# MiniXC/LightningFastSpeech2

Hardware: AMD Instinct MI355X
Metric: mel-frames/sec (whole node), 256-phoneme batch-32 (higher is better)
Workload: dtype bf16

## Files before the change

include/fs2.h:

```cpp
#ifndef FS2_H_
#define FS2_H_

#include <stddef.h>
#include <stdint.h>

#ifdef __cplusplus
extern "C" {
#endif

#define FS2_ABI_VERSION 4
#define FS2_MAX_LAYERS 32
#define FS2_MAX_VARIANCES 4
#define FS2_MAX_PRIORS 8
#define FS2_NAME_LEN 32

enum fs2_status {
    FS2_OK = 0,
    FS2_ERR_HIP = 1,
    FS2_ERR_SHAPE = 2,
    FS2_ERR_ARG = 3,
    FS2_ERR_WEIGHT = 4,
    FS2_ERR_STATE = 5,
    FS2_ERR_NOMEM = 6
};
// ... 77 lines not shown
int fs2_set_graphs(fs2_engine* e, int32_t on);
int64_t fs2_graph_replays(const fs2_engine* e);
int fs2_set_deferred_layernorm(fs2_engine* e, int32_t on);
int fs2_set_folded_layernorm(fs2_engine* e, int32_t on);
int fs2_set_tuning(fs2_engine* e, int32_t knob);
int fs2_force_buckets(fs2_engine* e, int32_t variance_index, const int32_t* idx_device);
int fs2_force_variance_targets(fs2_engine* e, int32_t variance_index, const float* target_device);
int fs2_debug_copy(fs2_engine* e, const char* what, void* dst_device, void* hip_stream);

enum fs2_kernel_class {
    FS2_K_CONV_GEMM = 0,
    FS2_K_GEMM = 1,
    FS2_K_ATTENTION = 2,
    FS2_K_ROWOPS = 3,
    FS2_K_DEC_FFN_CONV1 = 4,
    FS2_K_DEC_ATTENTION = 5,
    FS2_K_ENC_MHA = 6,
    FS2_K_PREDICTOR = 7,
    FS2_K_COUNT = 8
};
int fs2_profile_enable(fs2_engine* e, int32_t kernel_class, int32_t enable);
int fs2_profile_reserve(fs2_engine* e, int32_t kernel_class, int32_t pairs);
int fs2_profile_read(fs2_engine* e, int32_t kernel_class, double* total_ms, int64_t* launches,
                     double* flops, double* bytes);

int fs2_op_set_gemm_variant(int32_t variant);
int fs2_op_set_vocoder_lds_limit(int32_t kib);
int fs2_op_set_vocoder_fused_resblock(int32_t on);
int32_t fs2_op_vocoder_resblock_form(int32_t dtype, int32_t channels, int32_t taps, const int32_t* dilations, int32_t npairs);
int32_t fs2_op_vocoder_conv_tile(int32_t dtype, int32_t n, int32_t cin, int32_t taps, int32_t dil, int32_t shift, int32_t post,
                                 int32_t* cin_pad);
int fs2_op_gemm(int32_t dtype, int32_t out_dtype, const void* x, const void* w, const float* bias, void* c,
                int32_t M, int32_t N, int32_t Cin, int32_t taps, int32_t S, int32_t relu, void* hip_stream);
int fs2_op_gemm_relu_dropout(int32_t dtype, const void* x, const void* w, const float* bias, void* c, int32_t M, int32_t N, int32_t Cin,
                             int32_t taps, int32_t S, float p, uint64_t seed, uint64_t key, void* hip_stream);
int fs2_op_gemm_add(int32_t dtype, const void* x, const void* w, const float* bias, const void* addend, void* c, int32_t M, int32_t N,
                    int32_t Cin, int32_t taps, int32_t S, void* hip_stream);
int fs2_op_gemm_rowscale(const void* x, const void* w, const float* bias, const float* rowstats, const float* wg,
                         void* c, int32_t M, int32_t N, int32_t Cin, void* hip_stream);
int fs2_op_gemm_rowscale_dt(int32_t dtype, int32_t out_dtype, const void* x, const void* w, const float* bias, const float* rowstats,
                            const float* wg, void* c, int32_t M, int32_t N, int32_t Cin, void* hip_stream);
int fs2_op_gemm_stats(int32_t dtype, const void* x, const void* w, const float* bias, const void* res, void* c, float* stats, int32_t M,
                      int32_t N, int32_t Cin, int32_t relu, void* hip_stream);
int fs2_op_rowstats_finish(const float* parts, int32_t nparts, int32_t ncols, float eps, float* out, int32_t M, void* hip_stream);
int fs2_op_gemm_head(const void* x, const void* w, const float* bias, const float* head_gw, float* stats_out, float* head_out, int32_t M,
                     int32_t N, int32_t Cin, int32_t relu, void* hip_stream);
int fs2_op_head_finish(const float* parts, const float* dots, int32_t nparts, int32_t ncols, float eps, float sum_gw, float cst,
                       const uint8_t* mask, float* pred, int32_t M, void* hip_stream);
int fs2_op_gemm_splitk_choice(int32_t dtype, int32_t M, int32_t N, int32_t Cin, int32_t taps, int32_t S);
int32_t fs2_op_gemm_route(int32_t dtype, int32_t out_dtype, int32_t M, int32_t N, int32_t Cin, int32_t taps, int32_t S, int32_t ksplit,
                          uint32_t present, int32_t bias_aligned);
int fs2_op_gemm_splitk(int32_t dtype, int32_t out_dtype, const void* x, const void* w, void* c, float* part, int32_t M, int32_t N,
                       int32_t Cin, int32_t taps, int32_t S, int32_t ksplit, int32_t accumulate, void* hip_stream);
int fs2_op_gemm_gated(int32_t dtype, const void* x, const void* w, const float* bias, const void* gate, float scale, void* c,
                      int32_t M, int32_t N, int32_t Cin, int32_t taps, int32_t S, void* hip_stream);
int fs2_op_attention(int32_t dtype, const void* qkv, const uint8_t* key_pad_mask, void* out, void* vt_scratch,
                     uint64_t* bits_scratch, int32_t B, int32_t S, int32_t H, int32_t heads, void* hip_stream);
int fs2_op_attention_x3(const float* qkv, const uint8_t* key_pad_mask, float* out, void* split_scratch, uint64_t* bits_scratch,
                        int32_t B, int32_t S, int32_t H, int32_t heads, void* hip_stream);
int fs2_op_gemm_split_out(const void* x, const void* w, const float* bias, void* c_hi, void* c_lo, int32_t M, int32_t N, int32_t Cin,
                          int32_t split, void* hip_stream);
int fs2_op_gemm_ln(int32_t dtype, const void* x, const void* w, const float* bias, const void* res,
                   const float* ln_g, const float* ln_b, const float* dot_w, float dot_b, const uint8_t* mask,
                   float* pred, void* y, void* tmp, int32_t M, int32_t N, int32_t Cin, int32_t taps, int32_t S,
                   int32_t relu, void* hip_stream);
int fs2_op_gemm_ln_tape(int32_t dtype, const void* x, const void* w, const float* bias, const void* res, const float* ln_g,
// ... 251 lines not shown
```

lightningfastspeech2_amd/csrc/capi_ops.hip:

```cpp
#include <math.h>

#include "fs2_common.h"
#include "fs2_kernels.h"

using namespace fs2;

namespace fs2 {

template <typename S, typename D>
__global__ __launch_bounds__(256) void convert_kernel(const S* __restrict__ s, D* __restrict__ d, size_t n) {
    for (size_t i = (size_t)blockIdx.x * 256 + threadIdx.x; i < n; i += (size_t)gridDim.x * 256)
        d[i] = Num<D>::from_f32(Num<S>::to_f32(s[i]));
}

int launch_convert(const ConvertArgs& a, int sdt, int ddt, hipStream_t st) {
    if (a.n == 0) return FS2_OK;
    size_t blocks = (a.n + 255) / 256;
    if (blocks > 4096) blocks = 4096;
    const dim3 g((unsigned)blocks), b(256);
    if (sdt == FS2_F32 && ddt == FS2_F32) hipLaunchKernelGGL((convert_kernel<float, float>), g, b, 0, st, (const float*)a.src, (float*)a.dst, a.n);
    else if (sdt == FS2_F32 && ddt == FS2_BF16) hipLaunchKernelGGL((convert_kernel<float, bf16>), g, b, 0, st, (const float*)a.src, (bf16*)a.dst, a.n);
    else if (sdt == FS2_BF16 && ddt == FS2_F32) hipLaunchKernelGGL((convert_kernel<bf16, float>), g, b, 0, st, (const bf16*)a.src, (float*)a.dst, a.n);
    else if (sdt == FS2_BF16 && ddt == FS2_BF16) hipLaunchKernelGGL((convert_kernel<bf16, bf16>), g, b, 0, st, (const bf16*)a.src, (bf16*)a.dst, a.n);
    else if (sdt == FS2_F32 && ddt == FS2_F16) hipLaunchKernelGGL((convert_kernel<float, f16>), g, b, 0, st, (const float*)a.src, (f16*)a.dst, a.n);
    else if (sdt == FS2_F16 && ddt == FS2_F32) hipLaunchKernelGGL((convert_kernel<f16, float>), g, b, 0, st, (const f16*)a.src, (float*)a.dst, a.n);
    else if (sdt == FS2_F16 && ddt == FS2_F16) hipLaunchKernelGGL((convert_kernel<f16, f16>), g, b, 0, st, (const f16*)a.src, (f16*)a.dst, a.n);
    else return FS2_ERR_ARG;
    return hipGetLastError() == hipSuccess ? FS2_OK : FS2_ERR_HIP;
}

}

namespace fs2 {
int apply_knob(Tuning& t, int variant) {
    int ok = 1;
    if (variant == 1500 || variant == 1501) t.attn_x3 = variant - 1500;
    else if (variant >= 1400 && variant <= 1402) t.gemm_wres = variant - 1400;
    else if (variant == 1340 || variant == 1341) t.enc_attn_out = variant - 1340;
    else if (variant == 1320 || variant == 1321) t.pred_fuse_embed = variant - 1320;
    else if (variant >= 1200 && variant <= 1204) t.attn_pipe = variant - 1200;
    else if (variant == 1100 || variant == 1101) t.colsum_fused = variant - 1100;
    else if (variant == 1000 || variant == 1001) t.bgemm_tn256 = variant - 1000;
    else if (variant >= 905 && variant <= 908) { if (variant >= 907) t.attn_bwd_nb_dq = 3 + ((variant - 905) & 1); else t.attn_bwd_nb = 3 + ((variant - 905) & 1); }
    else if (variant == 909) t.attn_bwd_nb = 1;
    else if (variant >= 900 && variant <= 903) { if (variant >= 902) t.attn_bwd_nb_dq = ((variant - 900) & 1) + 1; else t.attn_bwd_nb = ((variant - 900) & 1) + 1; }
    else if (variant == 904) t.attn_bwd_nb_dq = 0;
    else if (variant == 800 || variant == 801) t.bgemm_full = variant - 800;
    else if (variant == 700 || variant == 701) t.bgemm_xcd = variant - 700;
    else if (variant == 500 || variant == 501) t.split_f32 = variant - 500;
    else if (variant == 230 || variant == 231) t.head_sums = variant - 230;
    else if (variant == 220 || variant == 221) t.gemm_persist = variant - 220;
    else if (variant >= 200 && variant <= 202) t.slab_xcd_remap = variant - 200;
    else if (variant >= 0 && variant <= 7 && variant != 2) t.gemm_variant = variant;
    else ok = 0;
    if (!ok) return FS2_ERR_ARG;
    ++t.gen;
    return FS2_OK;
}
Tuning& op_tuning() {
    static thread_local Tuning t;
    return t;
}
}

static GemmArgs gemm_args(const void* x, const void* w, const float* bias, void* c, int M, int N, int Cin, int taps, int S, int relu) {
    GemmArgs a;
    a.X = x; a.W = w; a.bias = bias; a.C = c;
    a.M = M; a.N = N; a.K = taps * Cin; a.ldx = Cin; a.ldc = N;
    a.Cin = Cin; a.taps = taps; a.pad = (taps - 1) / 2; a.S = S; a.relu = relu;
// ... 58 lines not shown
size_t fs2_op_masked_loss_ws_bytes(void) { return fs2::masked_loss_ws_bytes(); }

int fs2_op_masked_loss(const float* pred, const void* truth, int32_t truth_kind, const uint8_t* pad_mask, int64_t rows,
                       int32_t inner, int32_t kind, void* ws, float* out2, void* stream) {
    if (!pred || !truth || !pad_mask || !ws || !out2) return FS2_ERR_ARG;
    if ((kind != 0 && kind != 1) || (truth_kind != 0 && truth_kind != 1)) return FS2_ERR_ARG;
    fs2::LossArgs a;
    a.pred = pred; a.truth = truth; a.mask = pad_mask; a.ws = ws; a.out = out2;
    a.rows = rows; a.inner = inner; a.kind = kind; a.truth_kind = truth_kind;
    return fs2::launch_masked_loss(a, (hipStream_t)stream);
}

int fs2_op_set_vocoder_fused_resblock(int32_t on) {
    const bool defined = on == 0 || on == 1 || on == 2 || on == 4 || on == 7 || on == 9 || (on >= 50 && on <= 100);
    if (!defined) return FS2_ERR_ARG;
    fs2::op_tuning().voc_fused_resblock = on;
    return FS2_OK;
}

int fs2_op_set_vocoder_lds_limit(int32_t kib) {
    if (kib < 0 || kib > 150) return FS2_ERR_ARG;
    fs2::op_tuning().voc_lds_limit = kib;
    return FS2_OK;
}



int fs2_op_set_gemm_variant(int32_t variant) { return fs2::apply_knob(fs2::op_tuning(), variant); }

int fs2_op_gemm(int32_t dtype, int32_t out_dtype, const void* x, const void* w, const float* bias, void* c,
                int32_t M, int32_t N, int32_t Cin, int32_t taps, int32_t S, int32_t relu, void* stream) {
    GemmArgs a = gemm_args(x, w, bias, c, M, N, Cin, taps, S, relu);
    return launch_gemm(a, dtype, out_dtype, (hipStream_t)stream);
}

int fs2_op_gemm_relu_dropout(int32_t dtype, const void* x, const void* w, const float* bias, void* c, int32_t M, int32_t N, int32_t Cin,
                             int32_t taps, int32_t S, float p, uint64_t seed, uint64_t key, void* stream) {
    if (!(p > 0.f && p < 1.f)) return FS2_ERR_ARG;
    GemmArgs a = gemm_args(x, w, bias, c, M, N, Cin, taps, S, 1);
    a.drop_p = p; a.drop_seed = seed; a.drop_key = key;
    return launch_gemm(a, dtype, dtype, (hipStream_t)stream);
}

int fs2_op_gemm_add(int32_t dtype, const void* x, const void* w, const float* bias, const void* addend, void* c, int32_t M, int32_t N,
                    int32_t Cin, int32_t taps, int32_t S, void* stream) {
    if (!addend) return FS2_ERR_ARG;
    GemmArgs a = gemm_args(x, w, bias, c, M, N, Cin, taps, S, 0);
    a.epi_res = addend;
    if (N < 192 || M % S || !(taps & 1)) return FS2_ERR_SHAPE;
    return launch_gemm(a, dtype, dtype, (hipStream_t)stream);
}

int fs2_op_gemm_stats(int32_t dtype, const void* x, const void* w, const float* bias, const void* res, void* c, float* stats, int32_t M,
                      int32_t N, int32_t Cin, int32_t relu, void* stream) {
    if (!x || !w || !c || !stats) return FS2_ERR_ARG;
    GemmArgs a = gemm_args(x, w, bias, c, M, N, Cin, 1, M, relu);
    a.epi_res = res; a.stats_out = stats; a.ln_eps = 1e-5f;
    if (N < 192) return FS2_ERR_SHAPE;
    return launch_gemm(a, dtype, dtype, (hipStream_t)stream);
}

int fs2_op_gemm_rowscale(const void* x, const void* w, const float* bias, const float* rowstats, const float* wg,
                         void* c, int32_t M, int32_t N, int32_t Cin, void* stream) {
    return fs2_op_gemm_rowscale_dt(FS2_BF16, FS2_BF16, x, w, bias, rowstats, wg, c, M, N, Cin, stream);
}
int fs2_op_gemm_rowscale_dt(int32_t dtype, int32_t out_dtype, const void* x, const void* w, const float* bias, const float* rowstats,
// ... 474 lines not shown
```

lightningfastspeech2_amd/csrc/fs2_kernels.h:

```cpp
#pragma once
#include <hip/hip_runtime.h>
#include <stdint.h>

#include <type_traits>

#include "../../include/fs2.h"

namespace fs2 {

inline bool is_16bit(int dt) { return dt == FS2_BF16 || dt == FS2_F16; }
inline bool is_storage_dtype(int dt) { return dt == FS2_F32 || is_16bit(dt); }
inline bool is_f32_or_bf16(int dt) { return dt == FS2_F32 || dt == FS2_BF16; }
inline size_t elem_bytes(int dt) { return is_16bit(dt) ? 2 : 4; }

struct Tuning {
    int gemm_variant = 0;
    int gemm_wres = 1;
    int head_sums = 1;
    int gemm_persist = 1;
    int slab_xcd_remap = 1;
    int split_f32 = 0;
    int attn_pipe = 3;
    int attn_x3 = 1;
    int enc_attn_out = 1;
    int pred_fuse_embed = 1;
    int attn_bwd_nb = 1, attn_bwd_nb_dq = 0;
    int colsum_fused = 0;
    int bgemm_full = 1, bgemm_xcd = 1, bgemm_tn256 = 1;
    int voc_lds_limit = 0;
    int voc_fused_resblock = 1;
    unsigned long long gen = 0;
};
Tuning& op_tuning();
int apply_knob(Tuning& t, int variant);
inline const Tuning& tuning_of(const Tuning* t) { return t ? *t : op_tuning(); }

struct GemmArgs {
    const void* X;
    const void* W;
    const float* bias;
    void* C;
    void* C_lo = nullptr;
    int M, N, K;
    int ldx, ldc;
    int Cin, taps, pad;
    int S;
    int relu;
    const void* res = nullptr;
    const float* ln_g = nullptr;
    const float* ln_b = nullptr;
// ... 8 lines not shown
    const Tuning* tune = nullptr;
    const void* epi_res = nullptr;
    const float* epi_res_stats = nullptr;
    const float* epi_res_g = nullptr;
    const float* epi_res_b = nullptr;
    int epi_res_parts = 0;
    float* stats_out = nullptr;
    int w_presplit = 0;
    int split = 0;
    const uint8_t* zero_rows = nullptr;
    const void* gate = nullptr;
    float gate_scale = 1.f;
    float drop_p = 0.f;
    uint64_t drop_seed = 0, drop_key = 0;
    const float* rs_stats = nullptr;
    const float* rs_wg = nullptr;
    const float* head_gw = nullptr;
    float* head_out = nullptr;
    int ksplit = 0;
};
enum GemmFeature : unsigned {
    GF_BIAS = 1u << 0, GF_RES = 1u << 1, GF_LN = 1u << 2, GF_DOT = 1u << 3, GF_ZOUT = 1u << 4, GF_LNTMP = 1u << 5, GF_STATS = 1u << 6,
    GF_EPIRES = 1u << 7, GF_GATE = 1u << 8, GF_DROP = 1u << 9, GF_RS = 1u << 10 , GF_HEAD = 1u << 11 ,
    GF_ZR = 1u << 12, GF_CLO = 1u << 13, GF_SPLIT = 1u << 14, GF_WPRE = 1u << 15, GF_RELU = 1u << 16,
};
enum GemmFamily { GEMM_NONE = 0, GEMM_FLAT128 = 1, GEMM_SLAB = 2, GEMM_PERSIST = 3, GEMM_WRES = 4 };
struct GemmRoute {
    int status = FS2_OK;
    int family = GEMM_NONE;
    int mi = 0;
    int in_dtype = 0, out_dtype = 0;
    bool ln = false, split = false, defer = false, xpre = false;
    bool zr = false;
    bool two_launch = false;
    bool presplit = false;
};
inline bool layernorm_rows_ok(int H) { return H % 4 == 0 && H <= 1024; }
GemmRoute route_gemm(const GemmArgs& a, int in_dtype, int out_dtype);
int launch_route(const GemmRoute& r, const GemmArgs& a, hipStream_t stream);
inline int launch_gemm(const GemmArgs& a, int in_dtype, int out_dtype, hipStream_t stream) {
    return launch_route(route_gemm(a, in_dtype, out_dtype), a, stream);
}
int launch_presplit_pack(const float* w, void* out, size_t n_values, hipStream_t stream);
bool gemm_presplit_eligible(int N, int K);
int launch_split_k_reduce(const float* part, void* out, size_t n, int ksplit, int accumulate, int out_dtype, hipStream_t stream);
int gemm_splitk_choice(int M, int N, int Cin, int taps, int S, int in_dtype);
bool gemm_wres_supported(const GemmArgs& a, int in_dtype, int out_dtype, bool force);
int launch_gemm_wres(const GemmArgs& a, int dtype, hipStream_t stream);
bool gemm_persist_supported(const GemmArgs& a, int in_dtype, int out_dtype, int mi);
bool gemm_head_supported(const GemmArgs& a, int in_dtype, int out_dtype);
bool gemm_persist_pays(const GemmArgs& a, int mi);
int launch_gemm_persist(const GemmArgs& a, int dtype, int mi, hipStream_t stream);

struct AttnArgs {
    const void* qkv;
    void* vt;
    const uint64_t* kbits;
    void* out;
    int B, S, H, heads, Spad, nw64;
    float scale_log2e;
    const void* qkv_lo = nullptr;
    float* lse2 = nullptr;
    float drop_p = 0.f;
    uint64_t drop_seed = 0, drop_key = 0;
    const Tuning* tune = nullptr;
};
struct AttnOutArgs {
    const void* qkv;
    const uint64_t* kbits;
    const void* wpk;
    const float* bias;
    const void* res;
    const float* ln_g;
    const float* ln_b;
    void* out;
    int B, S, H, heads, nw64;
    float scale_log2e, eps;
};
bool attn_out_ln_supported(int dtype, int H, int heads, int S);
int launch_attn_out_ln(const AttnOutArgs& a, int dtype, hipStream_t stream);
struct AttnBwdArgs {
// ... 495 lines not shown
```

lightningfastspeech2_amd/csrc/gemm_mfma.hip:

```cpp
#include <string.h>

#include "fs2_common.h"
#include "fs2_kernels.h"

namespace fs2 {

static constexpr int BM = 128, BN = 128, ROWB = 128;
static constexpr int TILE_BYTES = BM * ROWB;

__device__ inline int swz(int row, int slot) { return row * ROWB + ((slot ^ (row & 7)) << 4); }

template <typename T, typename OutT, bool ZR = false>
__global__ __launch_bounds__(256) void gemm_conv_kernel(GemmArgs p) {
    extern __shared__ __attribute__((aligned(16))) unsigned char smem[];
    unsigned char* sX = smem;
    unsigned char* sW = smem + 2 * TILE_BYTES;
    constexpr int E16 = Num<T>::kPer16B;
    constexpr int KE = ROWB / (int)sizeof(T);

    const int tid = threadIdx.x, lane = tid & 63, wave = tid >> 6;
    const int tiles_n = (p.N + BN - 1) / BN;
    const int bm = blockIdx.x / tiles_n, bn = blockIdx.x % tiles_n;
    const int m0 = bm * BM, n0 = bn * BN;

// ... 1059 lines not shown
            mi = best;
        }
    }
    if (ln && family != GEMM_SLAB) return r;
    if (!rules_hold(q, subject, family)) return GemmRoute{FS2_ERR_SHAPE};
    r.family = family; r.mi = mi;
    if (family == GEMM_FLAT128) {
        r.zr = q.feats & GF_ZR;
        if (!(dtype_pair(in_dtype, out_dtype) & flat_dtypes(r.zr))) return GemmRoute{FS2_ERR_SHAPE};
    } else if (family == GEMM_SLAB) {
        r.ln = ln; r.defer = defer;
        if (!(dtype_pair(in_dtype, out_dtype) & slab_dtypes(ln, defer))) return GemmRoute{FS2_ERR_SHAPE};
        r.split = in_dtype == FS2_F32 && out_dtype == FS2_F32 && (q.have & ND_SPLIT_ON);
        r.xpre = r.split && a.taps > 1;
        r.presplit = r.split && !a.w_presplit;
    }
    return r;
}

static GemmRoute route_request(const GemmArgs& a, int in_dtype, int out_dtype) {
    const auto no = [](int status) { return GemmRoute{status}; };
    const auto on = [](int family, int mi) { GemmRoute r; r.family = family; r.mi = mi; return r; };
    if (!is_storage_dtype(in_dtype) || !is_storage_dtype(out_dtype)) return no(FS2_ERR_ARG);
    if ((in_dtype == FS2_F16 || out_dtype == FS2_F16) && (a.drop_p > 0.f || a.gate || a.z_out || a.ksplit > 1 || a.head_out || a.C_lo)) return no(FS2_ERR_ARG);
    const Tuning& tn = tuning_of(a.tune);
    if (a.head_out) {
        if (a.ln_g || !gemm_head_supported(a, in_dtype, out_dtype)) return no(FS2_ERR_SHAPE);
        return on(GEMM_PERSIST, 6);
    }
    if (!a.ln_g) {
        if (a.drop_p > 0.f) {
            if (!rules_hold(classify(a, in_dtype, out_dtype), GF_DROP, GEMM_NONE)) return no(FS2_ERR_SHAPE);
        } else if (tn.gemm_wres && tn.gemm_variant == 0 && a.ksplit <= 1 && gemm_wres_supported(a, in_dtype, out_dtype, tn.gemm_wres == 2)) {
            return on(GEMM_WRES, 0);
        }
        return route_one(a, in_dtype, out_dtype);
    }
    if (a.z_out && a.N > S_BN) return no(FS2_ERR_SHAPE);
    if (a.drop_p > 0.f && (a.N > S_BN || !a.z_out)) return no(FS2_ERR_SHAPE);
    if (a.N <= S_BN && in_dtype == out_dtype) {
        const GemmRoute r = route_one(a, in_dtype, out_dtype);
        if (r.status != FS2_OK || r.family != GEMM_NONE) return r;
    }
    if (a.z_out) return no(FS2_ERR_SHAPE);
    if (!a.ln_tmp || in_dtype != out_dtype) return no(FS2_ERR_ARG);
    GemmArgs g = a;
    g.ln_g = nullptr;
    g.C = a.ln_tmp;
    GemmRoute r = route_one(g, in_dtype, out_dtype);
    if (r.status != FS2_OK || r.family == GEMM_NONE) return r;
    if (!layernorm_rows_ok(a.N)) return no(FS2_ERR_SHAPE);
    r.two_launch = true;
    return r;
}
GemmRoute route_gemm(const GemmArgs& a, int in_dtype, int out_dtype) {
    GemmRoute r = route_request(a, in_dtype, out_dtype);
    r.in_dtype = in_dtype; r.out_dtype = out_dtype;
    return r;
}

template <int MI, bool LN, bool DEFER>
static int launch_slab_e(const GemmRoute& r, const GemmArgs& a, hipStream_t stream) {
    return with_dtypes<slab_dtypes(LN, DEFER)>(r.in_dtype, r.out_dtype, [&](auto t, auto o) {
        using T = typename decltype(t)::type;
        using OutT = typename decltype(o)::type;
        if constexpr (sizeof(T) == 4) {
            if (r.xpre) return launch_slab_t<T, OutT, MI, LN, true, DEFER, true>(a, stream);
            if (r.split) return launch_slab_t<T, OutT, MI, LN, true, DEFER>(a, stream);
        }
        return launch_slab_t<T, OutT, MI, LN, false, DEFER>(a, stream);
    });
}
template <int MI>
static int launch_slab_mi(const GemmRoute& r, const GemmArgs& a, hipStream_t stream) {
    if constexpr (MI <= 6) {
        if (r.ln) return launch_slab_e<MI, true, false>(r, a, stream);
        if (r.defer) return launch_slab_e<MI, false, true>(r, a, stream);
    }
    return launch_slab_e<MI, false, false>(r, a, stream);
}
template <bool ZR>
static int launch_flat(const GemmRoute& r, const GemmArgs& a, hipStream_t stream) {
    return with_dtypes<flat_dtypes(ZR)>(r.in_dtype, r.out_dtype, [&](auto t, auto o) {
        return launch_t<typename decltype(t)::type, typename decltype(o)::type, ZR>(a, stream);
    });
}

int launch_route(const GemmRoute& r, const GemmArgs& a_in, hipStream_t stream) {
    if (r.status != FS2_OK || r.family == GEMM_NONE) return r.status;
    GemmArgs a = a_in;
    if (r.two_launch) { a.ln_g = nullptr; a.C = a_in.ln_tmp; }
    void* tmp = nullptr;
    if (r.presplit) {
        const int st = presplit_on_the_fly(a, stream, &tmp);
        if (st != FS2_OK) { if (tmp) (void)hipFreeAsync(tmp, stream); return st; }
    }
    int st;
    if (r.family == GEMM_FLAT128) st = r.zr ? launch_flat<true>(r, a, stream) : launch_flat<false>(r, a, stream);
    else if (r.family == GEMM_PERSIST) st = launch_gemm_persist(a, r.in_dtype, r.mi, stream);
    else if (r.family == GEMM_WRES) st = launch_gemm_wres(a, r.in_dtype, stream);
    else if (r.mi == 1) st = launch_slab_mi<1>(r, a, stream);
    else if (r.mi == 2) st = launch_slab_mi<2>(r, a, stream);
    else if (r.mi == 4) st = launch_slab_mi<4>(r, a, stream);
    else if (r.mi == 6) st = launch_slab_mi<6>(r, a, stream);
    else st = launch_slab_mi<8>(r, a, stream);
    if (tmp) (void)hipFreeAsync(tmp, stream);
    if (st != FS2_OK || !r.two_launch) return st;
    LayerNormArgs l;
    l.x = a_in.ln_tmp; l.res = a_in.res; l.gamma = a_in.ln_g; l.beta = a_in.ln_b; l.y = a_in.C;
    l.dot_w = a_in.dot_w; l.dot_b = a_in.dot_b; l.mask = a_in.mask; l.pred = a_in.pred;
    l.M = a_in.M; l.H = a_in.N; l.eps = a_in.ln_eps;
    return launch_layernorm(l, r.out_dtype, stream);
}

bool gemm_presplit_eligible(int N, int K) { return N >= 192 && K % 32 == 0; }

__global__ __launch_bounds__(256) void presplit_pack_kernel(const float* w, unsigned char* out, size_t npairs) {
    const size_t i = (size_t)blockIdx.x * 256 + threadIdx.x;
    if (i >= npairs) return;
    const size_t chunk = i >> 2;
    const int sl = (int)(i & 3);
    const uint4 c0 = *(const uint4*)(w + chunk * 32 + 4 * sl), c1 = *(const uint4*)(w + chunk * 32 + 16 + 4 * sl);
    uint4 h, l;
    split_bf16x3(c0, c1, h, l);
    *(uint4*)(out + chunk * 128 + sl * 16) = h;
    *(uint4*)(out + chunk * 128 + (4 + sl) * 16) = l;
}
int launch_presplit_pack(const float* w, void* out, size_t n_values, hipStream_t stream) {
    if (n_values % 32) return FS2_ERR_SHAPE;
    if (!n_values) return FS2_OK;
    const size_t np = n_values / 8;
    hipLaunchKernelGGL(presplit_pack_kernel, dim3((unsigned)((np + 255) / 256)), dim3(256), 0, stream, w, (unsigned char*)out, np);
    return hipGetLastError() == hipSuccess ? FS2_OK : FS2_ERR_HIP;
// ... 58 lines not shown
```

lightningfastspeech2_amd/csrc/gemm_wres.hip:

```cpp
#include <hip/hip_runtime.h>

#include <type_traits>

#include "fs2_common.h"
#include "fs2_kernels.h"

namespace fs2 {
namespace {

constexpr int WR_K = 256, WR_ROWB = WR_K * 2, WR_MI = 3, WR_RT = 2 * WR_MI * 16;
constexpr int WR_TILEB = WR_RT * WR_ROWB;
__attribute__((unused)) constexpr int WR_NDMA = WR_TILEB / 1024 / 8;

__device__ __attribute__((unused)) inline int wr_wcol(int ni, int fgq) { return (ni >> 1) * 32 + fgq * 8 + (ni & 1) * 4; }

#ifdef FS2_WRES_PROBE
__device__ unsigned long long g_wres_stamps[2][64];
#define WRES_STAMP(i)                                                                                                      \
    do {                                                                                                                   \
        if (blockIdx.x == 0 && (threadIdx.x == 0 || threadIdx.x == 448) && (i) < 64)                                        \
            g_wres_stamps[threadIdx.x ? 1 : 0][i] = __builtin_amdgcn_s_memtime();                                           \
    } while (0)
#else
#define WRES_STAMP(i) do { } while (0)
#endif

template <typename T>
__global__ __launch_bounds__(512) void gemm_wres_kernel(GemmArgs p, int ncol, int nrg, int tiles) {
#if defined(__HIP_DEVICE_COMPILE__)
    __shared__ __attribute__((aligned(16))) unsigned char xs0[WR_TILEB];
    __shared__ __attribute__((aligned(16))) unsigned char xs1[WR_TILEB];
    const int tid = threadIdx.x, lane = tid & 63;
    const int wave = __builtin_amdgcn_readfirstlane(tid >> 6);
    const int wm = wave >> 2, wn = wave & 3, fr = lane & 15, fg = lane >> 4;
    const int xcd = blockIdx.x & 7, q = blockIdx.x >> 3;
    const int ct = q % ncol, rg = (q / ncol) * 8 + xcd;
    if (rg >= nrg) return;
    const int tbeg = (int)((long)rg * tiles / nrg), tend = (int)((long)(rg + 1) * tiles / nrg);
    if (tbeg >= tend) return;
    const int n0 = ct * 256;
    WRES_STAMP(0);

    uint4 fw[8][4];
    {
        const __amdgpu_buffer_rsrc_t wrs =
            __builtin_amdgcn_make_buffer_rsrc((void*)p.W, 0, (unsigned)((size_t)p.N * WR_K * 2), 0x00020000);
        auto wswz = [](int row) { return ((row >> 1) & 1) | (((row >> 3) & 3) << 1); };
        auto stage = [&](int cc0) {
#pragma unroll
            for (int c = 0; c < 2; ++c)
#pragma unroll
                for (int i = 0; i < 4; ++i) {
                    const int P = (i * 8 + wave) * 64 + lane, row = P >> 3, ps = P & 7;
                    const unsigned voff = (unsigned)((n0 + row) * (WR_K * 2) + (cc0 + c) * 128 + ((ps ^ wswz(row)) << 4));
                    __builtin_amdgcn_raw_ptr_buffer_load_lds(wrs, (__attribute__((address_space(3))) void*)((c ? xs1 : xs0) + (i * 8 + wave) * 1024),
                                                             16, voff, 0, 0, 0);
                }
            dma_drain();
            __syncthreads();
#pragma unroll
            for (int c = 0; c < 2; ++c)
#pragma unroll
                for (int ni = 0; ni < 4; ++ni) {
                    const int wrow = wn * 64 + wr_wcol(ni, fr >> 2) + (fr & 3);
#pragma unroll
                    for (int h = 0; h < 2; ++h)
                        fw[(cc0 + c) * 2 + h][ni] = *(const uint4*)((c ? xs1 : xs0) + wrow * 128 + (((h * 4 + fg) ^ wswz(wrow)) << 4));
                }
            __syncthreads();
        };
        stage(0);
        stage(2);
    }
    __shared__ __attribute__((aligned(16))) float sbias[256];
    if (tid < 256) sbias[tid] = p.bias ? p.bias[n0 + tid] : 0.f;
    __syncthreads();

    const __amdgpu_buffer_rsrc_t xrs =
        __builtin_amdgcn_make_buffer_rsrc((void*)p.X, 0, (unsigned)(((size_t)(p.M - 1) * p.ldx + WR_K) * 2), 0x00020000);
    auto issue_piece = [&](auto BUF, int t, int k, bool live) {
        unsigned char* const dst = decltype(BUF)::value ? xs1 : xs0;
        const int c = k * 8 + wave, i = 2 * c + (lane >> 5), ps = lane & 31, m = t * WR_RT + i;
        const int ls = (ps & 16) | ((((ps & 7) ^ (i & 7)) << 1) | ((ps >> 3) & 1));
        const unsigned voff = (live && m < p.M) ? (unsigned)m * (unsigned)(p.ldx * 2) + (unsigned)(ls << 4) : 0xFFFFF000u;
        __builtin_amdgcn_raw_ptr_buffer_load_lds(xrs, (__attribute__((address_space(3))) void*)(dst + c * 1024), 16, voff, 0, 0, 0);
    };
    auto issue = [&](auto BUF, int t) {
#pragma unroll
        for (int k = 0; k < WR_NDMA; ++k) issue_piece(BUF, t, k, true);
    };
    const int arow = (wm * (WR_MI * 16) + fr) * WR_ROWB;
    const int acx = (((fg & 1) << 3) | ((fg >> 1) ^ (fr & 7))) << 4;
    auto compute = [&](auto BUF, f32x4_t (&acc)[4][WR_MI], auto side) {
        const unsigned char* const xs = decltype(BUF)::value ? xs1 : xs0;
        uint4 fx[2][WR_MI];
        auto ldx = [&](uint4 (&f)[WR_MI], int ks) {
#pragma unroll
            for (int mi = 0; mi < WR_MI; ++mi)
                f[mi] = *(const uint4*)(xs + arow + mi * 16 * WR_ROWB + (acx ^ ((((ks & 3) << 1) | ((ks >> 2) << 4)) << 4)));
        };
        ldx(fx[0], 0);
#pragma unroll
        for (int ks = 0; ks < 8; ++ks) {
            if (ks + 1 < 8) ldx(fx[(ks + 1) & 1], ks + 1);
#pragma unroll
            for (int ni = 0; ni < 4; ++ni) {
#pragma unroll
                for (int mi = 0; mi < WR_MI; ++mi) Mma16<T>::step(fw[ks][ni], fx[ks & 1][mi], acc[ni][mi]);
                if (ni == 0) side(ks);
            }
        }
    };
    auto store_piece = [&](int t, int mi, int j, const uint4& q) {
        const int m = t * WR_RT + wm * (WR_MI * 16) + mi * 16 + fr;
        if (m < p.M) *(uint4*)((T*)p.C + (size_t)m * p.ldc + n0 + wn * 64 + j * 32 + fg * 8) = q;
    };
    using B0 = std::integral_constant<int, 0>;
    using B1 = std::integral_constant<int, 1>;
    WRES_STAMP(1);
    issue(B0{}, tbeg);
    auto tile = [&](auto CUR, auto NXT, int t) {
        WRES_STAMP(4 + (t - tbeg) * 5);
        if (t == tbeg) __builtin_amdgcn_s_waitcnt(0x0F70);
        else __builtin_amdgcn_s_waitcnt(0x0F70 | 6);
        WRES_STAMP(5 + (t - tbeg) * 5);
        __syncthreads();
        WRES_STAMP(6 + (t - tbeg) * 5);
        const bool has_next = t + 1 < tend;
        auto side = [&](int ks) {
            if (ks < WR_NDMA) issue_piece(NXT, t + 1, ks, has_next);
        };
        WRES_STAMP(7 + (t - tbeg) * 5);
        f32x4_t acc[4][WR_MI];
#pragma unroll
        for (int a = 0; a < 4; ++a)
#pragma unroll
            for (int b = 0; b < WR_MI; ++b) acc[a][b] = (f32x4_t){0.f, 0.f, 0.f, 0.f};
        compute(CUR, acc, side);
        WRES_STAMP(8 + (t - tbeg) * 5);
#pragma unroll
        for (int mi = 0; mi < WR_MI; ++mi) {
#pragma unroll
            for (int j = 0; j < 2; ++j) {
                const float4 b0 = *(const float4*)(sbias + wn * 64 + j * 32 + fg * 8), b1 = *(const float4*)(sbias + wn * 64 + j * 32 + fg * 8 + 4);
                const float bv[8] = {b0.x, b0.y, b0.z, b0.w, b1.x, b1.y, b1.z, b1.w};
                float v[8];
#pragma unroll
                for (int r = 0; r < 8; ++r) {
                    v[r] = acc[2 * j + (r >> 2)][mi][r & 3] + bv[r];
                    if (p.relu) v[r] = fmaxf(v[r], 0.f);
                }
                store_piece(t, mi, j, make_uint4(pack2<T>(v[0], v[1]), pack2<T>(v[2], v[3]), pack2<T>(v[4], v[5]), pack2<T>(v[6], v[7])));
            }
        }
    };
    for (int t = tbeg; t < tend; t += 2) {
        tile(B0{}, B1{}, t);
        if (t + 1 < tend) tile(B1{}, B0{}, t + 1);
    }
#else
    (void)p; (void)ncol; (void)nrg; (void)tiles;
#endif
}

}


static int wres_row_groups(int ncol, int tiles) {
    int nrg = (256 / ncol) & ~7;
    if (nrg < 8) nrg = 8;
    if (nrg > ((tiles + 7) & ~7)) nrg = (tiles + 7) & ~7;
    return nrg;
}

bool gemm_wres_supported(const GemmArgs& a, int in_dtype, int out_dtype, bool force) {
    if (a.N >= 256 && a.N % 256 == 0 && !force) {
        const int tiles = (a.M + WR_RT - 1) / WR_RT;
        if (tiles < 3 * wres_row_groups(a.N / 256, tiles)) return false;
    }
    return is_16bit(in_dtype) && out_dtype == in_dtype && a.taps == 1 && a.K == WR_K && a.Cin == WR_K && a.N >= 256 && a.N % 256 == 0 &&
           a.N <= 2048 && a.M > 0 && !a.res && !a.ln_g && !a.dot_w && !a.z_out && !a.epi_res && !a.stats_out && !a.gate && !a.zero_rows &&
           !a.split && !a.rs_stats && a.ldx % 8 == 0 && a.ldc % 8 == 0 && (size_t)a.M * a.ldx * 2 < 0xFFFFF000ull && (size_t)a.M * a.ldc * 2 < 0xFFFFF000ull;
}

int launch_gemm_wres(const GemmArgs& a, int dtype, hipStream_t stream) {
    if (!is_16bit(dtype)) return FS2_ERR_ARG;
    const int ncol = a.N / 256, tiles = (a.M + WR_RT - 1) / WR_RT, nrg = wres_row_groups(ncol, tiles);
    if (dtype == FS2_F16) hipLaunchKernelGGL(gemm_wres_kernel<f16>, dim3((unsigned)(nrg * ncol)), dim3(512), 0, stream, a, ncol, nrg, tiles);
    else hipLaunchKernelGGL(gemm_wres_kernel<bf16>, dim3((unsigned)(nrg * ncol)), dim3(512), 0, stream, a, ncol, nrg, tiles);
    return hipGetLastError() == hipSuccess ? FS2_OK : FS2_ERR_HIP;
}

}

#ifdef FS2_WRES_PROBE
extern "C" int fs2_dbg_wres_stamps(unsigned long long* out ) {
    if (hipDeviceSynchronize() != hipSuccess) return -1;
    return hipMemcpyFromSymbol(out, HIP_SYMBOL(fs2::g_wres_stamps), sizeof(unsigned long long) * 128) == hipSuccess ? 0 : -2;
}
#endif
```

Baseline: 26.72 million.

## Add wide 512-column weight-resident GEMM variant and buffer-store epilogue

Adds a wide mode to the weight-resident GEMM. Each block holds 512 output channels of weights in registers, every wave covers 64 columns, and the block makes two row passes per tile. This halves the number of column groups, so each X tile is streamed and staged in LDS fewer times. Stores now go through buffer-store instructions with out-of-range rows masked by offset, and dummy stores keep the vmcnt wait constant. The cost is more sequential compute per tile and fewer blocks, and the mode is on by default through a heuristic, with a new strided gemm entry point also added.

```diff
diff --git a/include/fs2.h b/include/fs2.h
--- a/include/fs2.h
+++ b/include/fs2.h
@@ -133,6 +133,8 @@
                                  int32_t* cin_pad);
 int fs2_op_gemm(int32_t dtype, int32_t out_dtype, const void* x, const void* w, const float* bias, void* c,
                 int32_t M, int32_t N, int32_t Cin, int32_t taps, int32_t S, int32_t relu, void* hip_stream);
+int fs2_op_gemm_ld(int32_t dtype, const void* x, const void* w, const float* bias, void* c, int32_t M, int32_t N, int32_t K,
+                   int32_t ldx, int32_t ldc, int32_t relu, void* hip_stream);
 int fs2_op_gemm_relu_dropout(int32_t dtype, const void* x, const void* w, const float* bias, void* c, int32_t M, int32_t N, int32_t Cin,
                              int32_t taps, int32_t S, float p, uint64_t seed, uint64_t key, void* hip_stream);
 int fs2_op_gemm_add(int32_t dtype, const void* x, const void* w, const float* bias, const void* addend, void* c, int32_t M, int32_t N,
diff --git a/lightningfastspeech2_amd/csrc/capi_ops.hip b/lightningfastspeech2_amd/csrc/capi_ops.hip
--- a/lightningfastspeech2_amd/csrc/capi_ops.hip
+++ b/lightningfastspeech2_amd/csrc/capi_ops.hip
@@ -35,6 +35,7 @@
 int apply_knob(Tuning& t, int variant) {
     int ok = 1;
     if (variant == 1500 || variant == 1501) t.attn_x3 = variant - 1500;
+    else if (variant >= 1410 && variant <= 1412) t.gemm_wres_wide = variant - 1410;
     else if (variant >= 1400 && variant <= 1402) t.gemm_wres = variant - 1400;
     else if (variant == 1340 || variant == 1341) t.enc_attn_out = variant - 1340;
     else if (variant == 1320 || variant == 1321) t.pred_fuse_embed = variant - 1320;
@@ -159,6 +160,14 @@
                 int32_t M, int32_t N, int32_t Cin, int32_t taps, int32_t S, int32_t relu, void* stream) {
     GemmArgs a = gemm_args(x, w, bias, c, M, N, Cin, taps, S, relu);
     return launch_gemm(a, dtype, out_dtype, (hipStream_t)stream);
+}
+
+int fs2_op_gemm_ld(int32_t dtype, const void* x, const void* w, const float* bias, void* c, int32_t M, int32_t N, int32_t K,
+                   int32_t ldx, int32_t ldc, int32_t relu, void* stream) {
+    if (ldx < K || ldc < N) return FS2_ERR_ARG;
+    GemmArgs a = gemm_args(x, w, bias, c, M, N, K, 1, M, relu);
+    a.ldx = ldx; a.ldc = ldc;
+    return launch_gemm(a, dtype, dtype, (hipStream_t)stream);
 }
 
 int fs2_op_gemm_relu_dropout(int32_t dtype, const void* x, const void* w, const float* bias, void* c, int32_t M, int32_t N, int32_t Cin,
diff --git a/lightningfastspeech2_amd/csrc/fs2_kernels.h b/lightningfastspeech2_amd/csrc/fs2_kernels.h
--- a/lightningfastspeech2_amd/csrc/fs2_kernels.h
+++ b/lightningfastspeech2_amd/csrc/fs2_kernels.h
@@ -16,6 +16,7 @@
 struct Tuning {
     int gemm_variant = 0;
     int gemm_wres = 1;
+    int gemm_wres_wide = 1;
     int head_sums = 1;
     int gemm_persist = 1;
     int slab_xcd_remap = 1;
@@ -90,6 +91,7 @@
     int in_dtype = 0, out_dtype = 0;
     bool ln = false, split = false, defer = false, xpre = false;
     bool zr = false;
+    bool wide = false;
     bool two_launch = false;
     bool presplit = false;
 };
@@ -104,7 +106,8 @@
 int launch_split_k_reduce(const float* part, void* out, size_t n, int ksplit, int accumulate, int out_dtype, hipStream_t stream);
 int gemm_splitk_choice(int M, int N, int Cin, int taps, int S, int in_dtype);
 bool gemm_wres_supported(const GemmArgs& a, int in_dtype, int out_dtype, bool force);
-int launch_gemm_wres(const GemmArgs& a, int dtype, hipStream_t stream);
+bool gemm_wres_wide_pays(const GemmArgs& a);
+int launch_gemm_wres(const GemmArgs& a, int dtype, bool wide, hipStream_t stream);
 bool gemm_persist_supported(const GemmArgs& a, int in_dtype, int out_dtype, int mi);
 bool gemm_head_supported(const GemmArgs& a, int in_dtype, int out_dtype);
 bool gemm_persist_pays(const GemmArgs& a, int mi);
diff --git a/lightningfastspeech2_amd/csrc/gemm_mfma.hip b/lightningfastspeech2_amd/csrc/gemm_mfma.hip
--- a/lightningfastspeech2_amd/csrc/gemm_mfma.hip
+++ b/lightningfastspeech2_amd/csrc/gemm_mfma.hip
@@ -1115,7 +1115,9 @@
         if (a.drop_p > 0.f) {
             if (!rules_hold(classify(a, in_dtype, out_dtype), GF_DROP, GEMM_NONE)) return no(FS2_ERR_SHAPE);
         } else if (tn.gemm_wres && tn.gemm_variant == 0 && a.ksplit <= 1 && gemm_wres_supported(a, in_dtype, out_dtype, tn.gemm_wres == 2)) {
-            return on(GEMM_WRES, 0);
+            GemmRoute r = on(GEMM_WRES, 0);
+            r.wide = tn.gemm_wres_wide == 2 ? a.N >= 512 : tn.gemm_wres_wide == 1 && gemm_wres_wide_pays(a);
+            return r;
         }
         return route_one(a, in_dtype, out_dtype);
     }
@@ -1181,7 +1183,7 @@
     int st;
     if (r.family == GEMM_FLAT128) st = r.zr ? launch_flat<true>(r, a, stream) : launch_flat<false>(r, a, stream);
     else if (r.family == GEMM_PERSIST) st = launch_gemm_persist(a, r.in_dtype, r.mi, stream);
-    else if (r.family == GEMM_WRES) st = launch_gemm_wres(a, r.in_dtype, stream);
+    else if (r.family == GEMM_WRES) st = launch_gemm_wres(a, r.in_dtype, r.wide, stream);
     else if (r.mi == 1) st = launch_slab_mi<1>(r, a, stream);
     else if (r.mi == 2) st = launch_slab_mi<2>(r, a, stream);
     else if (r.mi == 4) st = launch_slab_mi<4>(r, a, stream);
diff --git a/lightningfastspeech2_amd/csrc/gemm_wres.hip b/lightningfastspeech2_amd/csrc/gemm_wres.hip
--- a/lightningfastspeech2_amd/csrc/gemm_wres.hip
+++ b/lightningfastspeech2_amd/csrc/gemm_wres.hip
@@ -25,20 +25,15 @@
 #define WRES_STAMP(i) do { } while (0)
 #endif
 
-template <typename T>
-__global__ __launch_bounds__(512) void gemm_wres_kernel(GemmArgs p, int ncol, int nrg, int tiles) {
 #if defined(__HIP_DEVICE_COMPILE__)
-    __shared__ __attribute__((aligned(16))) unsigned char xs0[WR_TILEB];
-    __shared__ __attribute__((aligned(16))) unsigned char xs1[WR_TILEB];
+template <typename T, bool WIDE>
+__device__ __forceinline__ void wres_column_group(const GemmArgs& p, unsigned char (&xs0)[WR_TILEB], unsigned char (&xs1)[WR_TILEB],
+                                                  float (&sbias)[512], const int n0, const int tbeg, const int tend) {
+    constexpr int NPASS = WIDE ? 2 : 1;
+    constexpr int NSTORE = NPASS * WR_MI * 2;
     const int tid = threadIdx.x, lane = tid & 63;
     const int wave = __builtin_amdgcn_readfirstlane(tid >> 6);
-    const int wm = wave >> 2, wn = wave & 3, fr = lane & 15, fg = lane >> 4;
-    const int xcd = blockIdx.x & 7, q = blockIdx.x >> 3;
-    const int ct = q % ncol, rg = (q / ncol) * 8 + xcd;
-    if (rg >= nrg) return;
-    const int tbeg = (int)((long)rg * tiles / nrg), tend = (int)((long)(rg + 1) * tiles / nrg);
-    if (tbeg >= tend) return;
-    const int n0 = ct * 256;
+    const int wm = wave >> 2, wn = WIDE ? wave : wave & 3, fr = lane & 15, fg = lane >> 4;
     WRES_STAMP(0);
 
     uint4 fw[8][4];
@@ -46,34 +41,46 @@
         const __amdgpu_buffer_rsrc_t wrs =
             __builtin_amdgcn_make_buffer_rsrc((void*)p.W, 0, (unsigned)((size_t)p.N * WR_K * 2), 0x00020000);
         auto wswz = [](int row) { return ((row >> 1) & 1) | (((row >> 3) & 3) << 1); };
-        auto stage = [&](int cc0) {
+        auto stage = [&](int s) {
 #pragma unroll
             for (int c = 0; c < 2; ++c)
 #pragma unroll
                 for (int i = 0; i < 4; ++i) {
                     const int P = (i * 8 + wave) * 64 + lane, row = P >> 3, ps = P & 7;
-                    const unsigned voff = (unsigned)((n0 + row) * (WR_K * 2) + (cc0 + c) * 128 + ((ps ^ wswz(row)) << 4));
+                    const int chan = n0 + (WIDE ? c * 256 : 0) + row, chunk = WIDE ? s : 2 * s + c;
+                    const unsigned voff = (unsigned)(chan * (WR_K * 2) + chunk * 128 + ((ps ^ wswz(row)) << 4));
                     __builtin_amdgcn_raw_ptr_buffer_load_lds(wrs, (__attribute__((address_space(3))) void*)((c ? xs1 : xs0) + (i * 8 + wave) * 1024),
                                                              16, voff, 0, 0, 0);
                 }
             dma_drain();
             __syncthreads();
-#pragma unroll
-            for (int c = 0; c < 2; ++c)
-#pragma unroll
-                for (int ni = 0; ni < 4; ++ni) {
-                    const int wrow = wn * 64 + wr_wcol(ni, fr >> 2) + (fr & 3);
-#pragma unroll
-                    for (int h = 0; h < 2; ++h)
-                        fw[(cc0 + c) * 2 + h][ni] = *(const uint4*)((c ? xs1 : xs0) + wrow * 128 + (((h * 4 + fg) ^ wswz(wrow)) << 4));
-                }
+            const int wrow = (wave & 3) * 64 + (fr & 3);
+            if constexpr (WIDE) {
+                const unsigned char* const src = wm ? xs1 : xs0;
+#pragma unroll
+                for (int ni = 0; ni < 4; ++ni)
+#pragma unroll
+                    for (int h = 0; h < 2; ++h) {
+                        const int r = wrow + wr_wcol(ni, fr >> 2);
+                        fw[s * 2 + h][ni] = *(const uint4*)(src + r * 128 + (((h * 4 + fg) ^ wswz(r)) << 4));
+                    }
+            } else {
+#pragma unroll
+                for (int c = 0; c < 2; ++c)
+#pragma unroll
+                    for (int ni = 0; ni < 4; ++ni)
+#pragma unroll
+                        for (int h = 0; h < 2; ++h) {
+                            const int r = wrow + wr_wcol(ni, fr >> 2);
+                            fw[(2 * s + c) * 2 + h][ni] = *(const uint4*)((c ? xs1 : xs0) + r * 128 + (((h * 4 + fg) ^ wswz(r)) << 4));
+                        }
+            }
             __syncthreads();
         };
-        stage(0);
-        stage(2);
+#pragma unroll
+        for (int s = 0; s < (WIDE ? 4 : 2); ++s) stage(s);
     }
-    __shared__ __attribute__((aligned(16))) float sbias[256];
-    if (tid < 256) sbias[tid] = p.bias ? p.bias[n0 + tid] : 0.f;
+    if (WIDE || tid < 256) sbias[tid] = p.bias ? p.bias[n0 + tid] : 0.f;
     __syncthreads();
 
     const __amdgpu_buffer_rsrc_t xrs =
@@ -89,10 +96,10 @@
 #pragma unroll
         for (int k = 0; k < WR_NDMA; ++k) issue_piece(BUF, t, k, true);
     };
-    const int arow = (wm * (WR_MI * 16) + fr) * WR_ROWB;
     const int acx = (((fg & 1) << 3) | ((fg >> 1) ^ (fr & 7))) << 4;
-    auto compute = [&](auto BUF, f32x4_t (&acc)[4][WR_MI], auto side) {
+    auto compute = [&](auto BUF, const int rb, f32x4_t (&acc)[4][WR_MI], auto side) {
         const unsigned char* const xs = decltype(BUF)::value ? xs1 : xs0;
+        const int arow = (rb * (WR_MI * 16) + fr) * WR_ROWB;
         uint4 fx[2][WR_MI];
         auto ldx = [&](uint4 (&f)[WR_MI], int ks) {
 #pragma unroll
@@ -111,18 +118,27 @@
             }
         }
     };
-    auto store_piece = [&](int t, int mi, int j, const uint4& q) {
-        const int m = t * WR_RT + wm * (WR_MI * 16) + mi * 16 + fr;
-        if (m < p.M) *(uint4*)((T*)p.C + (size_t)m * p.ldc + n0 + wn * 64 + j * 32 + fg * 8) = q;
+    const __amdgpu_buffer_rsrc_t crs =
+        __builtin_amdgcn_make_buffer_rsrc((void*)p.C, 0, (unsigned)(((size_t)(p.M - 1) * p.ldc + p.N) * 2), 0x00020000);
+    typedef unsigned int u32x4_t __attribute__((ext_vector_type(4)));
+    const unsigned cbase = (unsigned)fr * (unsigned)(p.ldc * 2) + (unsigned)((n0 + wn * 64 + fg * 8) * 2);
+    auto store_piece = [&](int t, int rb, int mi, int j, const uint4& q) {
+        const int mrow = t * WR_RT + rb * (WR_MI * 16) + mi * 16;
+        const unsigned voff = fr < p.M - mrow ? cbase + ((unsigned)mrow * (unsigned)(p.ldc * 2) + (unsigned)(j * 64)) : 0xFFFFF000u;
+        __builtin_amdgcn_raw_buffer_store_b128((u32x4_t){q.x, q.y, q.z, q.w}, crs, voff, 0, 0);
+        __builtin_amdgcn_sched_barrier(0);
     };
     using B0 = std::integral_constant<int, 0>;
     using B1 = std::integral_constant<int, 1>;
     WRES_STAMP(1);
     issue(B0{}, tbeg);
+    __builtin_amdgcn_sched_barrier(0);
+#pragma unroll
+    for (int i = 0; i < NSTORE; ++i)
+        __builtin_amdgcn_raw_buffer_store_b128((u32x4_t){0u, 0u, 0u, 0u}, crs, 0xFFFFF000u + 16u * i, 0, 0);
     auto tile = [&](auto CUR, auto NXT, int t) {
         WRES_STAMP(4 + (t - tbeg) * 5);
-        if (t == tbeg) __builtin_amdgcn_s_waitcnt(0x0F70);
-        else __builtin_amdgcn_s_waitcnt(0x0F70 | 6);
+        __builtin_amdgcn_s_waitcnt(0x0F70 | NSTORE);
         WRES_STAMP(5 + (t - tbeg) * 5);
         __syncthreads();
         WRES_STAMP(6 + (t - tbeg) * 5);
@@ -131,26 +147,32 @@
             if (ks < WR_NDMA) issue_piece(NXT, t + 1, ks, has_next);
         };
         WRES_STAMP(7 + (t - tbeg) * 5);
-        f32x4_t acc[4][WR_MI];
-#pragma unroll
-        for (int a = 0; a < 4; ++a)
-#pragma unroll
-            for (int b = 0; b < WR_MI; ++b) acc[a][b] = (f32x4_t){0.f, 0.f, 0.f, 0.f};
-        compute(CUR, acc, side);
-        WRES_STAMP(8 + (t - tbeg) * 5);
-#pragma unroll
-        for (int mi = 0; mi < WR_MI; ++mi) {
-#pragma unroll
-            for (int j = 0; j < 2; ++j) {
-                const float4 b0 = *(const float4*)(sbias + wn * 64 + j * 32 + fg * 8), b1 = *(const float4*)(sbias + wn * 64 + j * 32 + fg * 8 + 4);
-                const float bv[8] = {b0.x, b0.y, b0.z, b0.w, b1.x, b1.y, b1.z, b1.w};
-                float v[8];
-#pragma unroll
-                for (int r = 0; r < 8; ++r) {
-                    v[r] = acc[2 * j + (r >> 2)][mi][r & 3] + bv[r];
-                    if (p.relu) v[r] = fmaxf(v[r], 0.f);
+#pragma unroll
+        for (int ps = 0; ps < NPASS; ++ps) {
+            const int rb = WIDE ? ps : wm;
+            f32x4_t acc[4][WR_MI];
+#pragma unroll
+            for (int a = 0; a < 4; ++a)
+#pragma unroll
+                for (int b = 0; b < WR_MI; ++b) acc[a][b] = (f32x4_t){0.f, 0.f, 0.f, 0.f};
+            if (ps == 0) compute(CUR, rb, acc, side);
+            else compute(CUR, rb, acc, [](int) {});
+            __builtin_amdgcn_sched_barrier(0);
+            WRES_STAMP(8 + (t - tbeg) * 5);
+#pragma unroll
+            for (int mi = 0; mi < WR_MI; ++mi) {
+#pragma unroll
+                for (int j = 0; j < 2; ++j) {
+                    const float4 b0 = *(const float4*)(sbias + wn * 64 + j * 32 + fg * 8), b1 = *(const float4*)(sbias + wn * 64 + j * 32 + fg * 8 + 4);
+                    const float bv[8] = {b0.x, b0.y, b0.z, b0.w, b1.x, b1.y, b1.z, b1.w};
+                    float v[8];
+#pragma unroll
+                    for (int r = 0; r < 8; ++r) {
+                        v[r] = acc[2 * j + (r >> 2)][mi][r & 3] + bv[r];
+                        if (p.relu) v[r] = fmaxf(v[r], 0.f);
+                    }
+                    store_piece(t, rb, mi, j, make_uint4(pack2<T>(v[0], v[1]), pack2<T>(v[2], v[3]), pack2<T>(v[4], v[5]), pack2<T>(v[6], v[7])));
                 }
-                store_piece(t, mi, j, make_uint4(pack2<T>(v[0], v[1]), pack2<T>(v[2], v[3]), pack2<T>(v[4], v[5]), pack2<T>(v[6], v[7])));
             }
         }
     };
@@ -158,8 +180,24 @@
         tile(B0{}, B1{}, t);
         if (t + 1 < tend) tile(B1{}, B0{}, t + 1);
     }
+}
+#endif
+
+template <typename T>
+__global__ __launch_bounds__(512) void gemm_wres_kernel(GemmArgs p, int nwide, int ncg, int nrg, int tiles) {
+#if defined(__HIP_DEVICE_COMPILE__)
+    __shared__ __attribute__((aligned(16))) unsigned char xs0[WR_TILEB];
+    __shared__ __attribute__((aligned(16))) unsigned char xs1[WR_TILEB];
+    __shared__ __attribute__((aligned(16))) float sbias[512];
+    const int xcd = blockIdx.x & 7, q = blockIdx.x >> 3;
+    const int ct = q % ncg, rg = (q / ncg) * 8 + xcd;
+    if (rg >= nrg) return;
+    const int tbeg = (int)((long)rg * tiles / nrg), tend = (int)((long)(rg + 1) * tiles / nrg);
+    if (tbeg >= tend) return;
+    if (ct < nwide) wres_column_group<T, true>(p, xs0, xs1, sbias, ct * 512, tbeg, tend);
+    else wres_column_group<T, false>(p, xs0, xs1, sbias, nwide * 512 + (ct - nwide) * 256, tbeg, tend);
 #else
-    (void)p; (void)ncol; (void)nrg; (void)tiles;
+    (void)p; (void)nwide; (void)ncg; (void)nrg; (void)tiles;
 #endif
 }
 
@@ -183,11 +221,24 @@
            !a.split && !a.rs_stats && a.ldx % 8 == 0 && a.ldc % 8 == 0 && (size_t)a.M * a.ldx * 2 < 0xFFFFF000ull && (size_t)a.M * a.ldc * 2 < 0xFFFFF000ull;
 }
 
-int launch_gemm_wres(const GemmArgs& a, int dtype, hipStream_t stream) {
+static int wres_column_groups(int N, bool wide, int* nwide) {
+    *nwide = wide ? N / 512 : 0;
+    return *nwide + (N - *nwide * 512) / 256;
+}
+
+bool gemm_wres_wide_pays(const GemmArgs& a) {
+    if (a.N < 512 || a.N % 512) return false;
+    int nwide;
+    const int tiles = (a.M + WR_RT - 1) / WR_RT, ncg = wres_column_groups(a.N, true, &nwide);
+    return tiles >= 3 * wres_row_groups(ncg, tiles);
+}
+
+int launch_gemm_wres(const GemmArgs& a, int dtype, bool wide, hipStream_t stream) {
     if (!is_16bit(dtype)) return FS2_ERR_ARG;
-    const int ncol = a.N / 256, tiles = (a.M + WR_RT - 1) / WR_RT, nrg = wres_row_groups(ncol, tiles);
-    if (dtype == FS2_F16) hipLaunchKernelGGL(gemm_wres_kernel<f16>, dim3((unsigned)(nrg * ncol)), dim3(512), 0, stream, a, ncol, nrg, tiles);
-    else hipLaunchKernelGGL(gemm_wres_kernel<bf16>, dim3((unsigned)(nrg * ncol)), dim3(512), 0, stream, a, ncol, nrg, tiles);
+    int nwide;
+    const int ncg = wres_column_groups(a.N, wide, &nwide), tiles = (a.M + WR_RT - 1) / WR_RT, nrg = wres_row_groups(ncg, tiles);
+    if (dtype == FS2_F16) hipLaunchKernelGGL(gemm_wres_kernel<f16>, dim3((unsigned)(nrg * ncg)), dim3(512), 0, stream, a, nwide, ncg, nrg, tiles);
+    else hipLaunchKernelGGL(gemm_wres_kernel<bf16>, dim3((unsigned)(nrg * ncg)), dim3(512), 0, stream, a, nwide, ncg, nrg, tiles);
     return hipGetLastError() == hipSuccess ? FS2_OK : FS2_ERR_HIP;
 }
 
```

Result: no change. 26.99 million (median of 4 runs) (+1.0%).
